# benbergner/ips

Measured on AMD Instinct MI355X. Metric: patches scored/sec (no-grad IPS loop), higher is better.
Workload: dtype f32; 1 GPU; Megapixel-MNIST 1500: 2500 patches of 1x32x32 per image (BASELINE configs[1]), B=16, M=64, I=64, n_token=4, use_pos, eager; parallelism=single GPU, dedup_blank=False, patch_storage=f32, loop_workgroups_per_image=1

## Files before the change

### ips_amd/csrc/scan_common.h

```cpp
#pragma once

#include <algorithm>
#include <cstdlib>

#include "ipsx_common.h"
#include "ipsx_math.h"
#include "ipsx_rowstats.h"
#include "ipsx_stdorder.h"

namespace ipsx {

typedef float f32x16 __attribute__((ext_vector_type(16)));

struct CandView {
    const float* cl;
    const float* lg;
    const int* cand;
    int R;
    __device__ __forceinline__ float get(int l, int r) const {
        if (cl) return cl[l * (R + 1) + r];
        const size_t row = cand ? (size_t)cand[l] : (size_t)l;
        return lg[row * R + r];
    }
};
// ... 714 lines not shown
    if (wave < nruns) {
        const int idx = wave * 64 + lane;
        mine = wave_sort_desc(idx < L ? src[idx] : 0ull, lane);
        runs[idx] = mine;
    }
    asm volatile("s_waitcnt lgkmcnt(0)\n\ts_barrier" ::: "memory");
    if (wave < nruns && mine != 0ull) {
        int rank = 0;
        int r0 = 0;
        for (; r0 + 8 <= nruns; r0 += 8) rank += rank_in_runs<8>(runs + r0 * 64, mine);
        const int left = nruns - r0;
        if (left >= 4) { rank += rank_in_runs<4>(runs + r0 * 64, mine); r0 += 4; }
        if (nruns - r0 == 3) rank += rank_in_runs<3>(runs + r0 * 64, mine);
        else if (nruns - r0 == 2) rank += rank_in_runs<2>(runs + r0 * 64, mine);
        else if (nruns - r0 == 1) rank += rank_in_runs<1>(runs + r0 * 64, mine);
        dst[rank] = mine;
    }
}

__device__ __forceinline__ void lds_barrier() { asm volatile("s_waitcnt lgkmcnt(0)\n\ts_barrier" ::: "memory"); }

#define FAST_STAMP(k)                                                              \
    do {                                                                           \
        if (STAMP) {                                                               \
            const unsigned long long t_ = __builtin_amdgcn_s_memtime();            \
            if (tid == 0) { tacc[k] += t_ - tlast; }                               \
            tlast = t_;                                                            \
        }                                                                          \
    } while (0)

__device__ __attribute__((noinline)) void tie_order_slow(uint64_t* sorted, uint64_t* other, int L, int m, int* stk) {
    torch_tie_order<SCAN_NT>(sorted, other, L, m, stk, threadIdx.x);
}

template <int R>
__device__ __forceinline__ void fold_row_max(uint32_t key, uint32_t* dst, int lane) {
    if (R <= 8) key = max(key, lane_xor_u32<8>(key, lane));
    if (R <= 16) key = max(key, lane_xor_u32<16>(key, lane));
    key = max(key, lane_xor_u32<32>(key, lane));
    if (lane < R && key != 0u) atomicMax(dst + lane, key);
}

__device__ __attribute__((noinline)) void exp_column(const float* xcol, float* ecol, int L, int ld, float mx) {
    for (int l = threadIdx.x; l < L; l += blockDim.x) ecol[l * ld] = det_expf_np(xcol[l * ld] - mx);
}

__device__ __attribute__((noinline)) void exp_column_part(const float* xcol, float* ecol, int L, int ld, float mx, int t0, int nt) {
    for (int l = t0; l < L; l += nt) ecol[l * ld] = det_expf_np(xcol[l * ld] - mx);
}

template <bool PERSIST>
__device__ __forceinline__ float scan_load(const float* p) {
    if (PERSIST) return __hip_atomic_load(p, __ATOMIC_RELAXED, __HIP_MEMORY_SCOPE_AGENT);
    return *p;
}

#define SCAN_WAIT_ROWS(need)                                                                                   \
    do {                                                                                                       \
        if (PERSIST && (long long)(need) > ready_known) {                                                      \
            if (wave == 0) {                                                                                   \
                unsigned long long t0_ = __builtin_amdgcn_s_memrealtime();                                     \
                int v_ = __hip_atomic_load(a.ready + b * a.ready_stride, __ATOMIC_RELAXED, __HIP_MEMORY_SCOPE_AGENT); \
                int seen_ = -1;                                                                                \
                while (v_ >= 0 && v_ < (need)) {                                                               \
                    __builtin_amdgcn_s_sleep(16);                                                              \
                    int w_ = lane < a.ready_words ? __hip_atomic_load(a.ready + lane, __ATOMIC_RELAXED, __HIP_MEMORY_SCOPE_AGENT) : 0; \
                    for (int o_ = 32; o_ >= 1; o_ >>= 1) w_ += __shfl_xor(w_, o_, 64);                         \
                    const unsigned long long now_ = __builtin_amdgcn_s_memrealtime();                          \
                    if (w_ != seen_) { seen_ = w_; t0_ = now_; }                                               \
                    if (now_ - t0_ > a.wait_ticks) { v_ = -1; break; }                                         \
                    v_ = __hip_atomic_load(a.ready + b * a.ready_stride, __ATOMIC_RELAXED, __HIP_MEMORY_SCOPE_AGENT); \
                }                                                                                              \
                if (lane == 0) ccount[6] = v_;                                                     \
            }                                                                                                  \
            lds_barrier();                                                                                     \
             \
             \
            __builtin_amdgcn_fence(__ATOMIC_ACQUIRE, "agent");                                                 \
            ready_known = ccount[6];                                                               \
            if (ready_known < 0) {                                                                             \
                if (tid == 0) { __hip_atomic_fetch_or(a.status, 1, __ATOMIC_RELAXED, __HIP_MEMORY_SCOPE_AGENT); a.plog[5] += 1; } \
                return;                                                                                        \
            }                                                                                                  \
        }                                                                                                      \
    } while (0)

template <int N, int J>
__device__ __forceinline__ uint32_t cmpx32(uint32_t s, uint32_t dir, int lane) {
    const uint32_t o = lane_xor_u32<J>(s, lane);
    const uint32_t c = (uint32_t)__builtin_amdgcn_sbfe((int)dir, N, 1);
    uint32_t d;
    asm("v_med3_u32 %0, %1, %2, %3" : "=v"(d) : "v"(s), "v"(o), "v"(c));
    return d;
}

__device__ __forceinline__ uint32_t sort_directions(int lane) {
    constexpr int KJ[21][2] = {{2, 1}, {4, 2}, {4, 1}, {8, 4}, {8, 2}, {8, 1}, {16, 8}, {16, 4}, {16, 2}, {16, 1}, {32, 16}, {32, 8},
                               {32, 4}, {32, 2}, {32, 1}, {64, 32}, {64, 16}, {64, 8}, {64, 4}, {64, 2}, {64, 1}};
    uint32_t d = 0u;
#pragma unroll
    for (int n = 0; n < 21; ++n) d |= ((((lane & KJ[n][0]) == 0) == ((lane & KJ[n][1]) == 0)) ? 1u : 0u) << n;
    return d;
}

__device__ __forceinline__ uint32_t wave_sort_desc_u32(uint32_t s, uint32_t dir, int lane) {
    s = cmpx32<0, 1>(s, dir, lane);
    s = cmpx32<1, 2>(s, dir, lane); s = cmpx32<2, 1>(s, dir, lane);
    s = cmpx32<3, 4>(s, dir, lane); s = cmpx32<4, 2>(s, dir, lane); s = cmpx32<5, 1>(s, dir, lane);
    s = cmpx32<6, 8>(s, dir, lane); s = cmpx32<7, 4>(s, dir, lane); s = cmpx32<8, 2>(s, dir, lane); s = cmpx32<9, 1>(s, dir, lane);
    s = cmpx32<10, 16>(s, dir, lane); s = cmpx32<11, 8>(s, dir, lane); s = cmpx32<12, 4>(s, dir, lane); s = cmpx32<13, 2>(s, dir, lane);
    s = cmpx32<14, 1>(s, dir, lane);
    s = cmpx32<15, 32>(s, dir, lane); s = cmpx32<16, 16>(s, dir, lane); s = cmpx32<17, 8>(s, dir, lane); s = cmpx32<18, 4>(s, dir, lane);
    s = cmpx32<19, 2>(s, dir, lane); s = cmpx32<20, 1>(s, dir, lane);
    return s;
}

struct TopmArgs {
    int tie_order, stk_off;
    const float* scores;
    int L, m, n2;
    long long* top;
    int* tie;
};

struct ScanCall {
    const float* logits;
    int b;
    int64_t n;
    int m, i, h, n_token;
    int64_t it_begin, it_end;
    int64_t* mem_idx;
    float* mem_score;
    int32_t* tie_flag;
    const int32_t* ready;
    int32_t* status;
    void* workspace;
    size_t workspace_bytes;
    void* stream;
    const int32_t* cond;
    int32_t cond_mask;
    int ready_stride, workgroups;
    int64_t logits_bstride_rows;
};

struct FastPlan {
    bool ok;
    int ept, lch;
    size_t lds;
};
FastPlan scan_fast_plan(int m, int i, int h, int n_token);
int launch_scan_fast(const ScanCall& c, const FastPlan& fp);
bool scan_cam_shape(int m, int i, int h, int n_token);
int launch_scan_cam(const ScanCall& c);
size_t scan_large_ws_per_image(int m, int i, int h, int n_token);
int launch_scan_large(const ScanCall& c);
int scan_large_team(int b, int m, int i, int h, int n_token);
int launch_topm_large(const TopmArgs& a, int b, void* workspace, size_t workspace_bytes, void* stream);
size_t topm_large_ws_per_row(int l);
int scan_large_max_l();

extern int g_persist_wait_ms;
extern bool g_scan_generic;
extern bool g_replay_stamps_on;
extern bool g_scan_direct;
extern bool g_scan_team_trunc;
extern int g_scan_team;
extern bool g_scan_r8;
extern unsigned long long* g_scan_stamps;
unsigned long long* persist_log();

inline int next_pow2(int v) { int p = 1; while (p < v) p <<= 1; return p; }
constexpr size_t kLdsLimit = 160 * 1024;

}
```

### ips_amd/csrc/scorer.hip

```cpp

#include <algorithm>
#include <cstdlib>

#include "scan_common.h"

namespace ipsx {

int g_tie_order = 1;
int g_persist_wait_ms = 50;
bool g_scan_generic = false;
bool g_replay_stamps_on = false;
bool g_scan_team_trunc = true;
int g_scan_team = -1;
bool g_scan_direct = true;
bool g_scan_r8 = true;
unsigned long long* g_scan_stamps = nullptr;

__device__ unsigned long long g_persist_log[8];


unsigned long long* persist_log() {
    static unsigned long long* p[64] = {nullptr};
    int dev = 0;
    if (hipGetDevice(&dev) != hipSuccess || dev < 0 || dev >= 64) dev = 0;
    if (!p[dev]) {
        void* q = nullptr;
        if (hipGetSymbolAddress(&q, HIP_SYMBOL(g_persist_log)) == hipSuccess) p[dev] = static_cast<unsigned long long*>(q);
    }
    return p[dev];
}

}

using namespace ipsx;

IPSX_API int ipsx_scan(const float* logits, int b, int64_t n, int m, int i, int h, int n_token,
                       int64_t* mem_idx, float* mem_score, int32_t* tie_flag, void* workspace, size_t workspace_bytes,
                       void* stream) {
    IPSX_REQUIRE(n > m && i > 0, "scan: needs more patches (%lld) than memory slots (%d)", (long long)n, m);
    if (tie_flag && hipMemsetAsync(tie_flag, 0, sizeof(int32_t) * (size_t)std::max(b, 0), as_stream(stream)) != hipSuccess)
        return fail(IPSX_EHIP, "scan: memset failed");
    return ipsx_scan_range(logits, b, n, m, i, h, n_token, 0, (n - m + i - 1) / i, mem_idx, mem_score, tie_flag,
                           workspace, workspace_bytes, stream);
}

static int scan_range_impl(const float* logits, int b, int64_t n, int m, int i, int h, int n_token,
                           int64_t it_begin, int64_t it_end, int64_t* mem_idx, float* mem_score,
                           int32_t* tie_flag, const int32_t* ready, int32_t* status, void* workspace,
                           size_t workspace_bytes, void* stream, const int32_t* cond = nullptr, int32_t cond_mask = 0,
                           int ready_stride = 0, int workgroups = 0, int64_t logits_bstride_rows = -1);

IPSX_API int ipsx_scan_range(const float* logits, int b, int64_t n, int m, int i, int h, int n_token,
                             int64_t it_begin, int64_t it_end, int64_t* mem_idx, float* mem_score,
                             int32_t* tie_flag, void* workspace, size_t workspace_bytes, void* stream) {
    return scan_range_impl(logits, b, n, m, i, h, n_token, it_begin, it_end, mem_idx, mem_score, tie_flag, nullptr, nullptr,
                           workspace, workspace_bytes, stream);
}

IPSX_API int ipsx_scan_range_strided(const float* logits, int64_t logits_bstride_rows, int b, int64_t n, int m, int i, int h,
                                     int n_token, int64_t it_begin, int64_t it_end, int64_t* mem_idx, float* mem_score,
                                     int32_t* tie_flag, void* workspace, size_t workspace_bytes, void* stream) {
    IPSX_REQUIRE(logits_bstride_rows >= n && logits_bstride_rows < ((int64_t)1 << 31),
                 "scan_range_strided: %lld rows between the images hold %lld candidates (fewer than 2^31)",
                 (long long)logits_bstride_rows, (long long)n);
    return scan_range_impl(logits, b, n, m, i, h, n_token, it_begin, it_end, mem_idx, mem_score, tie_flag, nullptr, nullptr,
                           workspace, workspace_bytes, stream, nullptr, 0, 0, 0, logits_bstride_rows);
}

IPSX_API size_t ipsx_scan_workspace_bytes(int b, int m, int i, int h, int n_token) {
    if (b <= 0 || m <= 0 || i <= 0 || h <= 0 || n_token <= 0) return 0;
    if (scan_fast_plan(m, i, h, n_token).ok && !g_scan_generic) return 0;
    return (size_t)b * scan_large_ws_per_image(m, i, h, n_token);
}

IPSX_API int ipsx_scan_workgroups_per_image(int b, int m, int i, int h, int n_token) {
    if (b <= 0 || m <= 0 || i <= 0 || h <= 0 || n_token <= 0) return 0;
    if (scan_fast_plan(m, i, h, n_token).ok && !g_scan_generic) return 1;
    return scan_large_team(b, m, i, h, n_token);
}

__global__ void publish_rows_kernel(int* ready, int value) {
    __hip_atomic_store(ready, value, __ATOMIC_RELEASE, __HIP_MEMORY_SCOPE_AGENT);
}

IPSX_API int ipsx_scan_persistent_supported(int m, int i, int h, int n_token) {
    if (m <= 0 || i <= 0 || h <= 0 || n_token <= 0) return 0;
    return scan_fast_plan(m, i, h, n_token).ok ? 1 : 0;
}

IPSX_API int ipsx_scan_persistent(const float* logits, int b, int64_t n, int m, int i, int h, int n_token,
                                  int64_t* mem_idx, float* mem_score, int32_t* tie_flag, const int32_t* ready,
                                  int32_t ready_per_image, int32_t* status, void* stream) {
    IPSX_REQUIRE(ready && status, "scan_persistent: needs the progress word(s) and the status word");
    IPSX_REQUIRE(n > m && i > 0, "scan: needs more patches (%lld) than memory slots (%d)", (long long)n, m);
    IPSX_REQUIRE(ipsx_scan_persistent_supported(m, i, h, n_token), "scan_persistent: shape not covered (use ipsx_scan_range)");
    return scan_range_impl(logits, b, n, m, i, h, n_token, 0, (n - m + i - 1) / i, mem_idx, mem_score, tie_flag, ready, status,
                           nullptr, 0, stream, nullptr, 0, ready_per_image ? 1 : 0);
}

IPSX_API int ipsx_scan_persistent_groupable(int m, int i, int h, int n_token) {
    return g_scan_r8 && scan_cam_shape(m, i, h, n_token) ? 1 : 0;
}

IPSX_API int ipsx_scan_persistent_on(const float* logits, int b, int64_t n, int m, int i, int h, int n_token,
                                     int64_t* mem_idx, float* mem_score, int32_t* tie_flag, const int32_t* ready,
                                     int32_t ready_per_image, int32_t* status, int workgroups, void* stream) {
    IPSX_REQUIRE(ready && status, "scan_persistent: needs the progress word(s) and the status word");
    IPSX_REQUIRE(n > m && i > 0, "scan: needs more patches (%lld) than memory slots (%d)", (long long)n, m);
    IPSX_REQUIRE(ipsx_scan_persistent_supported(m, i, h, n_token), "scan_persistent: shape not covered (use ipsx_scan_range)");
    return scan_range_impl(logits, b, n, m, i, h, n_token, 0, (n - m + i - 1) / i, mem_idx, mem_score, tie_flag, ready, status,
                           nullptr, 0, stream, nullptr, 0, ready_per_image ? 1 : 0, workgroups);
}

IPSX_API int ipsx_scan_persistent_ws(const float* logits, int b, int64_t n, int m, int i, int h, int n_token,
                                     int64_t* mem_idx, float* mem_score, int32_t* tie_flag, const int32_t* ready,
                                     int32_t ready_per_image, int32_t* status, int workgroups, void* workspace,
                                     size_t workspace_bytes, void* stream) {
    IPSX_REQUIRE(ready && status, "scan_persistent: needs the progress word(s) and the status word");
    IPSX_REQUIRE(n > m && i > 0, "scan: needs more patches (%lld) than memory slots (%d)", (long long)n, m);
    return scan_range_impl(logits, b, n, m, i, h, n_token, 0, (n - m + i - 1) / i, mem_idx, mem_score, tie_flag, ready, status,
                           workspace, workspace_bytes, stream, nullptr, 0, ready_per_image ? 1 : 0, workgroups);
}

IPSX_API int ipsx_scan_range_if_ws(const float* logits, int b, int64_t n, int m, int i, int h, int n_token,
                                   int64_t it_begin, int64_t it_end, int64_t* mem_idx, float* mem_score,
                                   int32_t* tie_flag, const int32_t* cond, int32_t cond_mask, void* workspace,
                                   size_t workspace_bytes, void* stream) {
    IPSX_REQUIRE(cond && cond_mask, "scan_range_if: needs the condition word and a mask");
    return scan_range_impl(logits, b, n, m, i, h, n_token, it_begin, it_end, mem_idx, mem_score, tie_flag, nullptr, nullptr,
                           workspace, workspace_bytes, stream, cond, cond_mask);
}

__global__ void scan_gate_kernel(const int* status, unsigned long long wait_ticks) {
    const unsigned long long t0 = __builtin_amdgcn_s_memrealtime();
    bool gave_up = false;
    while ((__hip_atomic_load(status, __ATOMIC_RELAXED, __HIP_MEMORY_SCOPE_AGENT) & 2) == 0) {
        __builtin_amdgcn_s_sleep(8);
        if (__builtin_amdgcn_s_memrealtime() - t0 > wait_ticks) { gave_up = true; break; }
    }
    const unsigned long long waited = __builtin_amdgcn_s_memrealtime() - t0;
    g_persist_log[0] += 1;
    g_persist_log[3] = t0;
    if (gave_up) g_persist_log[2] += 1;
    if (waited > g_persist_log[1]) {
        g_persist_log[1] = waited;
        g_persist_log[6] = t0;
        g_persist_log[7] = gave_up ? 0ull : __hip_atomic_load(&g_persist_log[4], __ATOMIC_RELAXED, __HIP_MEMORY_SCOPE_AGENT);
    }
}

IPSX_API int ipsx_scan_gate(const int32_t* status, void* stream) {
    IPSX_REQUIRE(status, "scan_gate: null pointer");
    scan_gate_kernel<<<dim3(1), dim3(1), 0, as_stream(stream)>>>(status, (unsigned long long)g_persist_wait_ms * 100000ull);
    return launched("scan_gate");
}

__global__ void part_wait_kernel(const int* done, int want, int* status, int bit, unsigned long long wait_ticks) {
    unsigned long long t0 = __builtin_amdgcn_s_memrealtime();
    int last = __hip_atomic_load(done, __ATOMIC_RELAXED, __HIP_MEMORY_SCOPE_AGENT);
    while (last < want) {
        __builtin_amdgcn_s_sleep(32);
        const int v = __hip_atomic_load(done, __ATOMIC_RELAXED, __HIP_MEMORY_SCOPE_AGENT);
        const unsigned long long t = __builtin_amdgcn_s_memrealtime();
        if (v != last) { last = v; t0 = t; }
        else if (t - t0 > wait_ticks) {
            __hip_atomic_fetch_or(status, bit, __ATOMIC_RELAXED, __HIP_MEMORY_SCOPE_AGENT);
            break;
        }
    }
    __builtin_amdgcn_fence(__ATOMIC_ACQUIRE, "agent");
}

IPSX_API int ipsx_part_wait(const int32_t* done, int32_t want, int32_t* status, int32_t bit, void* stream) {
    IPSX_REQUIRE(done && status && bit, "part_wait: needs the counter, the status word and a bit");
    part_wait_kernel<<<dim3(1), dim3(1), 0, as_stream(stream)>>>(done, want, status, bit,
                                                                 (unsigned long long)g_persist_wait_ms * 100000ull);
    return launched("part_wait");
}

IPSX_API int ipsx_publish_rows(int32_t* ready, int32_t value, void* stream) {
    IPSX_REQUIRE(ready, "publish_rows: null pointer");
    publish_rows_kernel<<<dim3(1), dim3(1), 0, as_stream(stream)>>>(ready, value);
    return launched("publish_rows");
}

IPSX_API int ipsx_scan_range_if(const float* logits, int b, int64_t n, int m, int i, int h, int n_token,
                                int64_t it_begin, int64_t it_end, int64_t* mem_idx, float* mem_score,
                                int32_t* tie_flag, const int32_t* cond, int32_t cond_mask, void* stream) {
    IPSX_REQUIRE(cond && cond_mask, "scan_range_if: needs the condition word and a mask");
    IPSX_REQUIRE(scan_fast_plan(m, i, h, n_token).ok, "scan_range_if: shapes of the LDS-resident loop only");
    return scan_range_impl(logits, b, n, m, i, h, n_token, it_begin, it_end, mem_idx, mem_score, tie_flag, nullptr, nullptr,
                           nullptr, 0, stream, cond, cond_mask);
}

static int scan_range_impl(const float* logits, int b, int64_t n, int m, int i, int h, int n_token,
                           int64_t it_begin, int64_t it_end, int64_t* mem_idx, float* mem_score,
                           int32_t* tie_flag, const int32_t* ready, int32_t* status, void* workspace,
                           size_t workspace_bytes, void* stream, const int32_t* cond, int32_t cond_mask, int ready_stride,
                           int workgroups, int64_t logits_bstride_rows) {
    IPSX_REQUIRE(logits && mem_idx, "scan: null pointer");
    IPSX_REQUIRE(b > 0 && m > 0 && i > 0 && h > 0 && n_token > 0, "scan: bad sizes");
    IPSX_REQUIRE(n > m, "scan: needs more patches (%lld) than memory slots (%d)", (long long)n, m);
    IPSX_REQUIRE(n < ((int64_t)1 << 31), "scan: too many patches");
    IPSX_REQUIRE(it_begin >= 0 && it_begin <= it_end && it_end <= (n - m + i - 1) / i,
                 "scan: iteration range [%lld, %lld) outside the loop", (long long)it_begin, (long long)it_end);
    if (it_begin == it_end) return IPSX_OK;
    const FastPlan fp = scan_fast_plan(m, i, h, n_token);
    ScanCall c = {logits, b, n, m, i, h, n_token, it_begin, it_end, mem_idx, mem_score, tie_flag, ready, status, workspace,
                  workspace_bytes, stream, cond, cond_mask, ready_stride, workgroups, logits_bstride_rows < 0 ? n : logits_bstride_rows};
    if (!fp.ok || (g_scan_generic && !ready && !cond)) return launch_scan_large(c);
    if (g_scan_r8 && scan_cam_shape(m, i, h, n_token)) return launch_scan_cam(c);
    return launch_scan_fast(c, fp);
}

IPSX_API int ipsx_set_persistent_wait_ms(int ms) {
    const int prev = g_persist_wait_ms;
    if (ms > 0) g_persist_wait_ms = ms > 20000 ? 20000 : ms;
    return prev;
}

IPSX_API int ipsx_set_tie_order(int mode) {
    const int prev = ipsx::g_tie_order;
    if (mode >= 0 && mode <= 2) ipsx::g_tie_order = mode;
    return prev;
}

extern "C" __attribute__((visibility("default"))) int ipsx_dbg_persist_log(unsigned long long* out8) {
    unsigned long long zero[8] = {0, 0, 0, 0, 0, 0, 0, 0};
    if (hipMemcpyFromSymbol(out8, HIP_SYMBOL(ipsx::g_persist_log), sizeof(zero)) != hipSuccess) return -1;
    return hipMemcpyToSymbol(HIP_SYMBOL(ipsx::g_persist_log), zero, sizeof(zero)) == hipSuccess ? 0 : -1;
}

extern "C" __attribute__((visibility("default"))) void ipsx_dbg_scan_stamps(unsigned long long* buf) {
    ipsx::g_scan_stamps = buf;
}

extern "C" __attribute__((visibility("default"))) void ipsx_dbg_scan_generic(int on) { g_scan_generic = on != 0; }

extern "C" __attribute__((visibility("default"))) void ipsx_dbg_scan_direct(int on) { g_scan_direct = on != 0; }
extern "C" __attribute__((visibility("default"))) void ipsx_dbg_scan_team(int w) { g_scan_team = w; }
extern "C" __attribute__((visibility("default"))) void ipsx_dbg_scan_team_trunc(int on) { g_scan_team_trunc = on != 0; }
extern "C" __attribute__((visibility("default"))) void ipsx_dbg_scan_r8(int on) { g_scan_r8 = on != 0; }
```

### ips_amd/dist.py

```python

import math

import torch
import torch.distributed as dist

from . import hip

PARTS = 4
DEFAULT_UNITS = 256

PART_SHARES = (0.5, 0.8, 0.95, 1.0)

PART_SHARES_LOOP_BOUND = (0.15, 0.4, 0.7, 1.0)


def part_iterations(n_iter, parts=PARTS, shares=None):
    P = max(1, min(parts, n_iter))
    shares = shares if shares is not None else PART_SHARES
    shares = shares if P == len(shares) else [(k + 1) / P for k in range(P)]
    its = [0]
    for k in range(P):
        lo = its[-1] + 1
        hi = n_iter - (P - 1 - k)
        its.append(min(max(round(shares[k] * n_iter), lo), hi))
    its[-1] = n_iter
    return its


class LaunchModel:

    REST_STEPS = ((0.25, 0.28), (0.5, 0.54), (0.75, 0.80), (1.0, 1.0))
    BESIDE = 3.5

    def __init__(self, round=0, t_round=0.0, t_row=0.0, t_launch=10.0, t_iter=7.0, t_xchg=60.0, kind="rows"):
        self.round, self.t_round, self.t_row = int(round), float(t_round), float(t_row)
        self.t_launch, self.t_iter, self.t_xchg, self.kind = float(t_launch), float(t_iter), float(t_xchg), kind

    def rounds(self, n):
        if n <= 0 or not self.round:
            return 0.0
        full, rest = divmod(int(n), self.round)
        if rest:
            f = rest / self.round
            full += next(c for lim, c in self.REST_STEPS if f <= lim)
        return float(full)

    def encode_us(self, n):
        if n <= 0:
            return 0.0
        return self.t_launch + (self.rounds(n) * self.t_round if self.round else n * self.t_row)

    def key(self):
        return (self.kind, self.round, round(self.t_round, 3), round(self.t_row, 6), self.t_launch, round(self.t_iter, 3), self.t_xchg)


def default_units():
    if torch.cuda.is_available():
        return hip.device_geometry(torch.device("cuda", torch.cuda.current_device())).cus
    return DEFAULT_UNITS


def loop_iteration_us(M, I, H, T):
    L, R = M + I, H * T
    if L > 1024:
        return 92.0 * L * R / 80000.0
    if (M, I, H, T) == (256, 256, 8, 1):
        return 4.2
    return 2.5 + L * R / 1000.0


_UNIT_FLOPS = 157.3e12 / 256


def _conv_macs(encoder, patch_shape):
    import copy
    macs = [0]

    def hook(m, inp, out):
        macs[0] += out[0].numel() * m.in_channels // m.groups * m.kernel_size[0] * m.kernel_size[1]
    try:
        enc = copy.deepcopy(encoder).to("meta").eval()
        hs = [m.register_forward_hook(hook) for m in enc.modules() if isinstance(m, torch.nn.Conv2d)]
        with torch.no_grad():
            enc(torch.empty((1,) + tuple(patch_shape[-3:]), device="meta"))
        for h in hs:
            h.remove()
    except Exception:
        return 100e6
    return float(macs[0])


def launch_model(net, patch_shape, units=None, precision=None):
    units = int(units or default_units())
    ca = net.transf.crs_attn
    t_iter = loop_iteration_us(net.M, net.I, ca.H, ca.n_token)
    precision = precision or hip.precision()
    if net.is_image and tuple(patch_shape[-3:]) == (1, 32, 32) and len(net.encoder) == 7:
        if precision == "bf16":
            return LaunchModel(round=16 * units, t_round=16 * 256 / 36.0, t_iter=t_iter, kind="fused32:bf16")
        t_round = {"fp32x3": 8 * 256 / 6.8}.get(precision, 8 * 37257216 / (_UNIT_FLOPS * 0.88) * 1e6)
        return LaunchModel(round=8 * units, t_round=t_round, t_iter=t_iter, kind="fused32:" + precision)
    if net.is_image:
        key = ("macs", tuple(patch_shape[-3:]))
        cache = net.__dict__.setdefault("_launch_model_cache", {})
        if key not in cache:
            cache[key] = _conv_macs(net.encoder, patch_shape)
        t_row = 2 * cache[key] / (_UNIT_FLOPS * units * 0.8) * 1e6
        n_conv = sum(1 for m in net.encoder.modules() if isinstance(m, torch.nn.Conv2d))
        return LaunchModel(t_row=t_row, t_launch=8.0 * n_conv, t_iter=t_iter, kind="layers")
    F = int(patch_shape[-1])
    return LaunchModel(t_row=2.0 * F * net.D / (_UNIT_FLOPS * units * 0.75) * 1e6, t_launch=15.0, t_iter=t_iter, kind="rows")


def _plan_cost(its, N, M, I, world, B, model):
    P = len(its) - 1
    done, main = [], 0.0
    for k in range(P):
        e0 = 0 if k == 0 else min(N, M + its[k] * I)
        e1 = N if k == P - 1 else min(N, M + its[k + 1] * I)
        main += model.encode_us(B * -(-(e1 - e0) // world))
        done.append(main)
    side = 0.0
    for k in range(P):
        side = max(side, done[k]) + model.t_xchg
        n = its[k + 1] - its[k]
        slow = model.t_iter * model.BESIDE
        beside = min(n, int(max(0.0, main - side) // slow))
        side += beside * slow + (n - beside) * model.t_iter
    return side


_PLAN_CACHE = {}


def plan_iterations(N, M, I, world, B=1, model=None, parts=PARTS):
    n_iter = math.ceil((N - M) / I)
    if model is None:
        return part_iterations(n_iter, parts)
    key = (N, M, I, world, B, parts, model.key())
    hit = _PLAN_CACHE.get(key)
    if hit is not None:
        return list(hit)
    cands = {tuple(part_iterations(n_iter, p, sh)) for p in range(1, parts + 1)
             for sh in (PART_SHARES, PART_SHARES_LOOP_BOUND, None)}
    if model.round:
        def piece(it0, it1):
            e0 = 0 if it0 == 0 else M + it0 * I
            return B * -(-(min(N, M + it1 * I) - e0) // world)

        def last_fitting(it0, limit):
            e0 = 0 if it0 == 0 else M + it0 * I
            rows = (limit // B) * world
            it1 = min((e0 + rows - M) // I, n_iter - 1)
            return it1 if it1 > it0 else None

        total_rounds = max(1.0, piece(0, n_iter) / model.round)

        def grow(prefix, left):
            cands.add(tuple(prefix + [n_iter]))
            if left <= 1:
                return
            it0 = prefix[-1]
            rest_rounds = piece(it0, n_iter) / model.round
            if rest_rounds <= 0.25:
                return
            limits = set()
            rs = range(0, int(rest_rounds) + 1)
            if len(rs) > 10:
                rs = sorted({int(round(rest_rounds * f)) for f in (0.08, 0.15, 0.25, 0.35, 0.5, 0.65, 0.8, 0.9, 0.95)} |
                            {1, 2, int(rest_rounds) - 1, int(rest_rounds)})
            for r in rs:
                for frac, _ in ((0.0, 0.0),) + (LaunchModel.REST_STEPS[:3] if total_rounds < 6 else ()):
                    lim = int((r + frac) * model.round)
                    if lim > 0:
                        limits.add(lim)
            nxt = {last_fitting(it0, lim) for lim in limits}
            for it1 in sorted(x for x in nxt if x is not None):
                grow(prefix + [it1], left - 1)

        grow([0], parts)
    best = min(cands, key=lambda c: (round(_plan_cost(c, N, M, I, world, B, model), 3), len(c), c))
    _PLAN_CACHE[key] = best
    return list(best)


def partition(N, M, I, world, parts=PARTS, B=1, model=None):
    its = plan_iterations(N, M, I, world, B, model, parts)
    P = len(its) - 1
    edges = [0] + [min(N, M + it * I) for it in its[1:]]
    edges[-1] = N
    piece = [max(1, math.ceil((edges[k + 1] - edges[k]) / world)) for k in range(P)]
    return its, edges, piece


class ShardPlan:

    def __init__(self, N, M, I, world, B=1, model=None, parts=PARTS):
        self.N, self.M, self.I, self.world, self.B, self.model = N, M, I, world, B, model
        self.its, self.edges, self.piece = partition(N, M, I, world, parts, B, model)

    def spans(self, rank):
        out = []
        for k, q in enumerate(self.piece):
            lo = min(self.edges[k] + rank * q, self.edges[k + 1])
            out.append((lo, min(lo + q, self.edges[k + 1])))
        return out

    def indices(self, rank):
        spans = self.spans(rank)
        return torch.cat([torch.arange(lo, hi, dtype=torch.int64) for lo, hi in spans]) if spans else torch.empty(0, dtype=torch.int64)

    def launches(self, rank):
        return [self.B * (hi - lo) for lo, hi in self.spans(rank)]

    def rounds(self, rank=0):
        n = self.launches(rank)
        if self.model is None or not self.model.round:
            return 0.0, 0.0
        return sum(self.model.rounds(v) for v in n), sum(n) / self.model.round

# ... 310 lines not shown
```

### ips_amd/hip.py

```python

import collections
import ctypes as C
import os
import subprocess

import torch

_PKG = os.path.dirname(os.path.abspath(__file__))
_SO = os.path.join(_PKG, "lib", "libipsx.so")
_LIB = None

f32p = C.c_void_p
ABI_MAJOR = 3


def backend():
    b = os.environ.get("IPSX_BACKEND", "hip").lower()
    if b not in ("hip", "aten"):
        raise ValueError("IPSX_BACKEND must be 'hip' or 'aten', got {!r}".format(b))
    return b


def precision():
    p = os.environ.get("IPSX_PRECISION", "fp32").lower()
# ... 618 lines not shown
    if len(tables):
        held, held_rows, piece, dst = tables[0]
        if piece is not None:
            raise ValueError("table 0 is the patch table: its piece is the view (pass None)")
        if dst.dtype != images.dtype or tuple(dst.shape[2:]) != view.patch_shape or dst.device != images.device:
            raise ValueError("table 0: rows of {} {}, the view's patches are {} {}".format(
                dst.dtype, tuple(dst.shape[2:]), images.dtype, view.patch_shape))
    arr, B = _stream_tables(tables, n_cand)
    if sel is not None and (sel.dtype != torch.int64 or tuple(sel.shape) != (B, M) or not sel.is_contiguous()):
        raise ValueError("sel must be a contiguous (B, M) int64 tensor")
    unit = C.c_int(0)
    st = _stream() if images.is_cuda else None
    _ck(lib().ipsx_stream_commit_view(arr, len(tables), _p(images), C.byref(view.struct), images.element_size(), _p(sel), B or 0,
                                      M, n_cand, tail_first, C.byref(unit), st), "ipsx_stream_commit_view")
    return unit.value


def scan_range_if(lg, M, I, H, T, it_begin, it_end, mem_idx, tie, cond, mask=1, workspace=None):
    B, N = lg.shape[:2]
    if workspace is not None:
        _ck(lib().ipsx_scan_range_if_ws(_p(lg), B, N, M, I, H, T, it_begin, it_end, _p(mem_idx), None, _p(tie), _p(cond), mask,
                                        _p(workspace), workspace.numel(), _stream()), "ipsx_scan_range_if_ws")
        return mem_idx
    _ck(lib().ipsx_scan_range_if(_p(lg), B, N, M, I, H, T, it_begin, it_end, _p(mem_idx), None, _p(tie), _p(cond), mask,
                                 _stream()), "ipsx_scan_range_if")
    return mem_idx


Geometry = collections.namedtuple("Geometry", "cus xcds cus_per_xcd")
_GEOMETRY = {}


def device_geometry(dev):
    dev = torch.device(dev)
    idx = dev.index if dev.index is not None else torch.cuda.current_device()
    g = _GEOMETRY.get(idx)
    if g is None:
        props = torch.cuda.get_device_properties(idx)
        cus = int(props.multi_processor_count)
        arch = str(getattr(props, "gcnArchName", ""))
        xcds = cus // 32 if (arch.startswith("gfx95") or arch.startswith("gfx94")) and cus % 32 == 0 and cus >= 32 else 1
        g = _GEOMETRY[idx] = Geometry(cus, xcds, cus // xcds)
    return g


_PERSIST_OK = {}
_PERSIST_OFF = None


def persistent_wait_ms(ms=0):
    return lib().ipsx_set_persistent_wait_ms(int(ms))


_PERSIST_STRIKES = 0
_PERSIST_WAIT_SET = False


def persistent_ok(dev):
    global _PERSIST_WAIT_SET
    if _PERSIST_OFF is not None:
        return False
    if not _PERSIST_WAIT_SET:
        _PERSIST_WAIT_SET = True
        ms = int(os.environ.get("IPSX_PERSIST_WAIT_MS", "0") or 0)
        if ms > 0:
            persistent_wait_ms(ms)
    dev = torch.device(dev)
    idx = dev.index if dev.index is not None else torch.cuda.current_device()
    ok = _PERSIST_OK.get(idx)
    if ok is None:
        ok = _PERSIST_OK[idx] = _persistent_selftest(torch.device("cuda", idx))
    return ok


def persistent_disable(reason):
    global _PERSIST_OFF
    if _PERSIST_OFF is None:
        import warnings
        _PERSIST_OFF = reason
        warnings.warn("ips_amd: persistent selection loops are switched off for this process: " + reason +
                      " (IPSX_SCAN_PERSIST=0 avoids the attempt)")


_PERSIST_CALLS = 0
_PERSIST_RECENT = []


def persistent_timed_out(dev):
    global _PERSIST_STRIKES
    import warnings
    _PERSIST_STRIKES += 1
    limit = max(1, int(os.environ.get("IPSX_PERSIST_STRIKES", "3") or 3))
    window = max(1, int(os.environ.get("IPSX_PERSIST_WINDOW", "1000") or 1000))
    _PERSIST_RECENT[:] = [c for c in _PERSIST_RECENT if _PERSIST_CALLS - c < window] + [_PERSIST_CALLS]
    what = "a persistent selection loop timed out waiting for rows (its call was redone with per-part launches: results valid)"
    if len(_PERSIST_RECENT) >= limit:
        persistent_disable("%s - %d such events within %d calls" % (what, len(_PERSIST_RECENT), window))
        return False
    dev = torch.device(dev)
    idx = dev.index if dev.index is not None else torch.cuda.current_device()
    ok = _PERSIST_OK[idx] = _persistent_selftest(torch.device("cuda", idx))
    if not ok:
        persistent_disable(what + "; a loop beside its producer no longer passes the device's self-test")
        return False
    warnings.warn("ips_amd: %s; the device's self-test passes, the persistent pipelines stay on (event %d of %d allowed within "
                  "%d calls; IPSX_PERSIST_WAIT_MS raises the wait, IPSX_PERSIST_STRIKES the allowance)"
                  % (what, len(_PERSIST_RECENT), limit, window))
    return True


def _persistent_selftest(dev):
    M = I = 16
    H, T = 8, 1
    if not scan_persistent_supported(M, I, H, T):
        return False
    N = M + 4 * I
    with torch.cuda.device(dev):
        lg = torch.zeros((1, N, H * T), dtype=torch.float32, device=dev)
        mem = torch.empty((1, M), dtype=torch.int64, device=dev)
        words = torch.zeros((3,), dtype=torch.int32, device=dev)
        side, main = side_stream(dev), torch.cuda.current_stream(dev)
        side.wait_stream(main)
        with torch.cuda.stream(side):
            scan_persistent(lg, M, I, H, T, mem, words[0:1], words[1:2], words[2:3])
        scan_gate(words[2:3])
        publish_rows(words[1:2], N)
        main.wait_stream(side)
        torch.cuda.synchronize(dev)
        status = int(words[2].item())
    return (status & 1) == 0 and (status & 2) == 2


_SIDE_STREAMS = {}


def side_stream(dev):
    dev = torch.device(dev)
    key = (dev.type, dev.index if dev.index is not None else torch.cuda.current_device())
    st = _SIDE_STREAMS.get(key)
    if st is None:
        st = _SIDE_STREAMS[key] = torch.cuda.Stream(device=dev, priority=-1)
    return st


def scan_persistent_supported(M, I, H, T):
    return bool(lib().ipsx_scan_persistent_supported(M, I, H, T))


def scan_persistent_large(M, I, H, T):
    return (not scan_persistent_supported(M, I, H, T) and lib().ipsx_scan_workspace_bytes(1, M, I, H, T) > 0
            and M + I <= 16384 and H * T <= 256)


def scan_persistent_groupable(M, I, H, T):
    return bool(lib().ipsx_scan_persistent_groupable(M, I, H, T))


def scan_persistent(lg, M, I, H, T, mem_idx, tie, ready, status, workgroups=0, workspace=None, stream=None):
    B, N = lg.shape[:2]
    if not lg.is_contiguous():
        raise ValueError("scan_persistent needs the full contiguous (B, N, H*T) logits buffer")
    if ready.numel() not in (1, B):
        raise ValueError("ready: one word, or one per image")
    st = C.c_void_p(stream.cuda_stream) if stream is not None else _stream()
    if workspace is not None:
        _ck(lib().ipsx_scan_persistent_ws(_p(lg), B, N, M, I, H, T, _p(mem_idx), None, _p(tie), _p(ready),
                                          1 if (ready.numel() == B and B > 1) else 0, _p(status), int(workgroups),
                                          _p(workspace), workspace.numel(), st), "ipsx_scan_persistent_ws")
        return mem_idx
    _ck(lib().ipsx_scan_persistent_on(_p(lg), B, N, M, I, H, T, _p(mem_idx), None, _p(tie), _p(ready),
                                      1 if (ready.numel() == B and B > 1) else 0, _p(status), int(workgroups), st),
        "ipsx_scan_persistent_on")
    return mem_idx


def scan_gate(status):
    _ck(lib().ipsx_scan_gate(_p(status), _stream()), "ipsx_scan_gate")


def publish_rows(ready, n_rows):
    _ck(lib().ipsx_publish_rows(_p(ready), int(n_rows), _stream()), "ipsx_publish_rows")


def _scores_impl(x, qs, wk, H, Dk, T, want_attn):
    x = _f32(x)
    B, L, D = x.shape
    sc = torch.empty((B, L), dtype=torch.float32, device=x.device)
    attn = torch.empty((B, H, T, L), dtype=torch.float32, device=x.device) if want_attn else None
    nb = lib().ipsx_scores_workspace_bytes(B, L, D, H, T)
    ws = torch.empty(max(nb, 1), dtype=torch.uint8, device=x.device)
    wkp = pack_linear(wk)
    _ck(lib().ipsx_scores(_p(x), _p(wkp), _p(qs), B, L, D, H, Dk, T, _p(sc), _p(attn),
                          _p(ws), nb, _stream()), "ipsx_scores")
    return sc, attn


def scores(x, qs, wk, H, Dk, T):
    return _scores_impl(x, qs, wk, H, Dk, T, False)[0]


def attn_map(x, qs, wk, H, Dk, T):
    return _scores_impl(x, qs, wk, H, Dk, T, True)[1]


def topm(sc, M):
    sc = _f32(sc)
    B, L = sc.shape
    top = torch.empty((B, M), dtype=torch.int64, device=sc.device)
    tie = torch.zeros((B,), dtype=torch.int32, device=sc.device)
    nb = lib().ipsx_topm_workspace_bytes(B, L, M)
    ws = torch.empty(nb, dtype=torch.uint8, device=sc.device) if nb else None
    _ck(lib().ipsx_topm(_p(sc), B, L, M, _p(top), _p(tie), _p(ws), nb, _stream()), "ipsx_topm")
    return top


def gather_rows(src, idx):
    B, M = idx.shape
    if src.stride(0) == 0 and src.shape[0] > 1:
        src = src[:1]
    src = src if src.is_contiguous() else src.contiguous()
    idx = idx if idx.is_contiguous() else idx.contiguous()
    N = src.shape[1]
    row_bytes = src[0, 0].numel() * src.element_size()
    out = torch.empty((B, M) + tuple(src.shape[2:]), dtype=src.dtype, device=src.device)
    bstride = N if src.shape[0] > 1 else 0
    _ck(lib().ipsx_gather_rows(_p(src), _p(idx), _p(out), B, N, M, row_bytes, bstride, _stream()),
        "ipsx_gather_rows")
    return out


def dequant_patches(q, table):
    if q.dtype != torch.uint8 or q.dim() < 3:
        raise TypeError("expected uint8 (..., C, h, w) patches, got {} {}".format(q.dtype, tuple(q.shape)))
    table = _patch_table(table, q.shape[-3], q.device)
    q = q if q.is_contiguous() else q.contiguous()
    out = torch.empty(q.shape, dtype=torch.float32, device=q.device)
    c, hw = q.shape[-3], q.shape[-2] * q.shape[-1]
    _ck(lib().ipsx_dequant_patches(_p(q), _p(table), _p(out), q.numel() // max(1, c * hw), c, hw, _stream()),
        "ipsx_dequant_patches")
    return out


def ips_finish_supported(src, pos):
    if not (on_device(src) and src.is_contiguous() and src.dim() >= 3):
        return False
    if (src[0, 0].numel() * src.element_size()) % 16 or src.data_ptr() % 16:
        return False
    if pos is None:
        return True
    if not on_device(pos) or pos.dim() != 3:
        return False
    p1 = pos[:1] if pos.stride(0) == 0 else pos
    return p1.is_contiguous() and (pos.shape[2] * pos.element_size()) % 16 == 0 and pos.data_ptr() % 16 == 0


def ips_finish(src, pos, idx_buf, status, status_host, order=None):
    B, M = idx_buf.shape
    N = src.shape[1]
    row_bytes = src[0, 0].numel() * src.element_size()
    out = torch.empty((B, M) + tuple(src.shape[2:]), dtype=src.dtype, device=src.device)
    idx = torch.empty_like(idx_buf)
    out_pos = None
    pos_bytes = pos_bs = 0
    if pos is not None:
        pos_bs = 0 if (pos.stride(0) == 0 or pos.shape[0] == 1) else pos.shape[1]
        pos_bytes = pos.shape[2] * pos.element_size()
        out_pos = torch.empty((B, M, pos.shape[2]), dtype=pos.dtype, device=pos.device)
    if order is not None:
        if order.dtype != torch.int64 or order.dim() != 2 or order.shape[1] != N or order.shape[0] not in (1, B) or \
                not order.is_contiguous() or order.device != src.device:
            raise ValueError("order must be a contiguous (B or 1, N) int64 tensor on the patches' device")
        _ck(lib().ipsx_ips_finish_indexed(_p(src), row_bytes, N if src.shape[0] > 1 else 0, N, _p(pos), pos_bytes, pos_bs, _p(idx_buf),
                                          _p(order), N if order.shape[0] > 1 else 0, B, M, _p(out), _p(out_pos), _p(idx), _p(status),
                                          _p(status_host), _stream()), "ipsx_ips_finish_indexed")
        return idx, out, out_pos
    _ck(lib().ipsx_ips_finish(_p(src), row_bytes, N if src.shape[0] > 1 else 0, N, _p(pos), pos_bytes, pos_bs, _p(idx_buf), B, M,
                              _p(out), _p(out_pos), _p(idx), _p(status), _p(status_host), _stream()), "ipsx_ips_finish")
    return idx, out, out_pos


def order_index(order, B, N, out=None):
    if order.dtype != torch.int64 or order.dim() != 2 or order.shape[1] != N or order.shape[0] not in (1, B) or \
            not order.is_contiguous() or not order.is_cuda:
        raise ValueError("order must be a contiguous (B or 1, N) int64 tensor on the device")
    if out is None:
        out = torch.empty((B, N), dtype=torch.int32, device=order.device)
    elif out.dtype != torch.int32 or out.numel() != B * N or not out.is_contiguous() or out.device != order.device:
        raise ValueError("out must be B * N contiguous int32 on the order's device")
    _ck(lib().ipsx_order_index(_p(order), N if order.shape[0] > 1 else 0, B, N, _p(out), _stream()), "ipsx_order_index")
    return out.view(B, N)


def patchify(img, patch_size, patch_stride):
    img = _f32(img)
    B, Cc, H, W = img.shape
    (ph, pw), (sh, sw) = patch_size, patch_stride
    n = lib().ipsx_patchify_count(H, W, ph, pw, sh, sw)
    if n <= 0:
        raise ValueError("patch {}x{} / stride {}x{} does not fit a {}x{} image".format(ph, pw, sh, sw, H, W))
    out = torch.empty((B, n, Cc, ph, pw), dtype=torch.float32, device=img.device)
    _ck(lib().ipsx_patchify(_p(img), B, Cc, H, W, ph, pw, sh, sw, _p(out), _stream()), "ipsx_patchify")
    return out


class PatchView:

# ... 178 lines not shown
```

Baseline: 34.01 million patches/s.

## Add shape-specialized scan kernel for M=I=64, 8 heads x 4 tokens

Adds a dedicated single-workgroup-per-image iterative top-M scan kernel, hard-coded for M=I=64, H=8, T=4 (the Megapixel-MNIST config). Inside the loop it double-buffers the logits and their exponentials in LDS and recomputes exp only for columns whose row max changed. Ranking is a counting sort with 8 threads per key. Half the workgroup prefetches the next chunk while the other half scores. The dispatcher routes matching shapes to it by default, and the loop-time cost model gets a fixed per-iteration estimate for this shape. It adds a large specialized code path that must match the generic kernel's tie-handling semantics.

Result: faster. 38.52 million patches/s, median of 6 (+13.3%).

```diff
diff --git a/ips_amd/csrc/scan_common.h b/ips_amd/csrc/scan_common.h
--- a/ips_amd/csrc/scan_common.h
+++ b/ips_amd/csrc/scan_common.h
@@ -890,6 +890,8 @@
 int launch_scan_fast(const ScanCall& c, const FastPlan& fp);
 bool scan_cam_shape(int m, int i, int h, int n_token);
 int launch_scan_cam(const ScanCall& c);
+bool scan_mnist_shape(int m, int i, int h, int n_token);
+int launch_scan_mnist(const ScanCall& c);
 size_t scan_large_ws_per_image(int m, int i, int h, int n_token);
 int launch_scan_large(const ScanCall& c);
 int scan_large_team(int b, int m, int i, int h, int n_token);
@@ -904,6 +906,7 @@
 extern bool g_scan_team_trunc;
 extern int g_scan_team;
 extern bool g_scan_r8;
+extern bool g_scan_mnist;
 extern unsigned long long* g_scan_stamps;
 unsigned long long* persist_log();
 
diff --git a/ips_amd/csrc/scan_mnist.hip b/ips_amd/csrc/scan_mnist.hip
--- /dev/null
+++ b/ips_amd/csrc/scan_mnist.hip
@@ -0,0 +1,311 @@
+
+#include <algorithm>
+#include <cstdlib>
+
+#include "scan_common.h"
+
+namespace ipsx {
+
+namespace mn {
+constexpr int M = 64, I = 64, L = 128, R = 32, H = 8, T = 4, LD = 36, NT = 1024;
+constexpr int OFF_KEYA = 0;
+constexpr int OFF_SORTED = OFF_KEYA + L * 8;
+constexpr int OFF_CAND = OFF_SORTED + L * 8;
+constexpr int OFF_PMAX = OFF_CAND + 2 * L * 4;
+constexpr int OFF_CNT = OFF_PMAX + 4 * R * 4;
+constexpr int OFF_PREV = OFF_CNT + 32;
+constexpr int OFF_DEN = OFF_PREV + 2 * R * 4;
+constexpr int OFF_X = (OFF_DEN + R * 4 + 15) & ~15;
+constexpr int OFF_E = OFF_X + 2 * L * LD * 4;
+constexpr int OFF_STK = OFF_E + 2 * L * LD * 4;
+constexpr int LDS_BYTES = OFF_STK + STK_BYTES;
+static_assert(OFF_KEYA % 16 == 0 && OFF_X % 16 == 0 && (LD * 4) % 16 == 0, "16-byte rows");
+static_assert(H * T == R && M + I == L && L * 8 == NT, "scan_mnist_kernel: 8 threads per key");
+static_assert(OFF_STK == 77728, "scan_mnist_kernel: 77,728 B of LDS + the replay's scratch (STK_BYTES)");
+static_assert(LDS_BYTES <= 160 * 1024, "scan_mnist_kernel: LDS");
+}
+
+template <int K>
+__device__ __forceinline__ float quad_bcast(float v) {
+    return as_float((uint32_t)__builtin_amdgcn_update_dpp(0, (int)as_u32(v), K * 0x55, 0xF, 0xF, false));
+}
+
+template <bool PERSIST>
+__global__ __launch_bounds__(mn::NT) void scan_mnist_kernel(ScanArgs a) {
+    using namespace mn;
+    extern __shared__ __attribute__((aligned(16))) unsigned char smem[];
+    if (!PERSIST && scan_skipped(a.cond, a.cond_mask)) return;
+    __builtin_amdgcn_s_setprio(3);
+    if (PERSIST) {
+        asm volatile("v_mov_b32 v127, 0" ::: "v127");
+        if (threadIdx.x == 0) {
+            __hip_atomic_fetch_or(a.status, 2, __ATOMIC_RELAXED, __HIP_MEMORY_SCOPE_AGENT);
+            __hip_atomic_store(&a.plog[4], (unsigned long long)__builtin_amdgcn_s_memrealtime(), __ATOMIC_RELAXED, __HIP_MEMORY_SCOPE_AGENT);
+        }
+    }
+    uint64_t* const keyA = reinterpret_cast<uint64_t*>(smem + OFF_KEYA);
+    uint64_t* const sorted = reinterpret_cast<uint64_t*>(smem + OFF_SORTED);
+    uint32_t* const pmax = reinterpret_cast<uint32_t*>(smem + OFF_PMAX);
+    int* const ccount = reinterpret_cast<int*>(smem + OFF_CNT);
+    uint32_t* const prevk = reinterpret_cast<uint32_t*>(smem + OFF_PREV);
+    float* const rden = reinterpret_cast<float*>(smem + OFF_DEN);
+    const int tid = threadIdx.x, lane = tid & 63, wave = tid >> 6;
+    const int b = blockIdx.x;
+    const int r = tid & (R - 1);
+    const int hid = tid - 512;
+    const float* const lg = a.lg + (size_t)b * a.n * R;
+    int ready_known = 0;
+    if (tid < 4 * R) pmax[tid] = 0u;
+    if (tid < 2) ccount[2 + tid] = 0;
+    lds_barrier();
+    SCAN_WAIT_ROWS(std::min<long long>(a.n, a.it0 * (long long)I + M + I));
+    {
+        float* const x0 = reinterpret_cast<float*>(smem + OFF_X);
+        int* const cand0 = reinterpret_cast<int*>(smem + OFF_CAND);
+        uint32_t km = 0u;
+#pragma unroll
+        for (int k = 0; k < 2; ++k) {
+            const int l = (tid >> 5) + 32 * k;
+            const size_t row = a.it0 == 0 ? (size_t)l : (size_t)a.mem_idx[(size_t)b * M + l];
+            const float v = scan_load<PERSIST>(lg + row * R + r);
+            x0[l * LD + r] = v;
+            km = max(km, max_key(v));
+        }
+        fold_row_max<R>(km, pmax, lane);
+        if (tid < M) cand0[tid] = a.it0 == 0 ? tid : (int)a.mem_idx[(size_t)b * M + tid];
+    }
+    const long long n_iter = a.it1 - a.it0;
+    float pf[4];
+    {
+        float* const x0 = reinterpret_cast<float*>(smem + OFF_X);
+        int* const cand0 = reinterpret_cast<int*>(smem + OFF_CAND);
+        const long long lo = a.it0 * (long long)I + M;
+        const int cnt = n_iter > 0 ? (int)std::min<long long>(I, a.n - lo) : 0;
+        uint32_t kc = 0u;
+#pragma unroll
+        for (int k = 0; k < 2; ++k) {
+            const int e = tid + NT * k;
+            if (e < cnt * R) {
+                const float v = scan_load<PERSIST>(lg + (size_t)lo * R + e);
+                x0[(M + (e >> 5)) * LD + r] = v;
+                kc = max(kc, max_key(v));
+            }
+        }
+        fold_row_max<R>(kc, pmax + R, lane);
+        if (tid < cnt) cand0[M + tid] = (int)(lo + tid);
+        const long long lo1 = lo + I;
+        const int cnt1 = n_iter > 1 ? (int)std::max<long long>(0, std::min<long long>(I, a.n - lo1)) : 0;
+        if (cnt1 > 0) SCAN_WAIT_ROWS(lo1 + cnt1);
+#pragma unroll
+        for (int k = 0; k < 4; ++k) {
+            const int e = hid + 512 * k;
+            pf[k] = (hid >= 0 && e < cnt1 * R) ? scan_load<PERSIST>(lg + (size_t)lo1 * R + e) : 0.0f;
+        }
+    }
+    int tie = 0;
+    const int n_it = (int)n_iter, n_rows = (int)a.n;
+    for (int k_it = 0; k_it < n_it; ++k_it) {
+        const int lo = ((int)a.it0 + k_it) * I + M;
+        const int cnt = min(I, n_rows - lo);
+        const int Lc = M + cnt;
+        const int par = k_it & 1;
+        float* const xc = reinterpret_cast<float*>(smem + OFF_X) + par * (L * LD);
+        float* const xn = reinterpret_cast<float*>(smem + OFF_X) + (par ^ 1) * (L * LD);
+        float* const ec = reinterpret_cast<float*>(smem + OFF_E) + par * (L * LD);
+        float* const en = reinterpret_cast<float*>(smem + OFF_E) + (par ^ 1) * (L * LD);
+        int* const cand = reinterpret_cast<int*>(smem + OFF_CAND) + par * L;
+        int* const cnew = reinterpret_cast<int*>(smem + OFF_CAND) + (par ^ 1) * L;
+        uint32_t* const mkey = pmax + 2 * R * par;
+        uint32_t* const mkey_nx = pmax + 2 * R * (par ^ 1);
+        const int lo1 = lo + I;
+        const int cnt1 = k_it + 1 < n_it ? max(0, min(I, n_rows - lo1)) : 0;
+        lds_barrier();
+        if (tid == 0) ccount[2 + (par ^ 1)] = 0;
+        const uint32_t mbits = as_u32(max_key_value(max(mkey[r], mkey[R + r])));
+        const float rowmax = as_float(mbits);
+        const bool changed = k_it == 0 || prevk[par * R + r] != mbits;
+        if (tid < R) prevk[(par ^ 1) * R + r] = mbits;
+        {
+            unsigned long long moved = __ballot(changed) & 0xFFFFFFFFull;
+            if (moved != 0ull) {
+                if (__popcll(moved) >= 8) {
+                    if (changed) {
+#pragma unroll
+                        for (int k = 0; k < 4; ++k) {
+                            const int l = (tid >> 5) + 32 * k;
+                            if (l < Lc) ec[l * LD + r] = det_expf_np(xc[l * LD + r] - rowmax);
+                        }
+                    }
+                } else {
+                    while (moved) {
+                        const int rr = __ffsll((long long)moved) - 1;
+                        moved &= moved - 1ull;
+                        exp_column(xc + rr, ec + rr, Lc, LD, __shfl(rowmax, rr, 64));
+                    }
+                }
+                lds_barrier();
+            }
+        }
+        {
+            const float* const col = ec + lane * LD + wave;
+            const float a0 = col[0], a1 = col[64 * LD], b0 = col[16], b1 = col[64 * LD + 16];
+            const bool has1 = lane + 64 < Lc;
+            float s0 = 0.0f, s1 = 0.0f;
+            s0 = s0 + a0; s1 = s1 + b0;
+            s0 = s0 + (has1 ? a1 : 0.0f); s1 = s1 + (has1 ? b1 : 0.0f);
+            wave_sum2(s0, s1, lane);
+            if (lane == 0) { rden[wave] = 1.0f / s0; rden[wave + 16] = 1.0f / s1; }
+        }
+        lds_barrier();
+        if (tid < 2 * R) mkey[tid] = 0u;
+        if (wave < 8) {
+            const int l = tid >> 2, t = tid & 3;
+            const float* const er = ec + l * LD + t;
+            float ev[H], dn[H];
+#pragma unroll
+            for (int hh = 0; hh < H; ++hh) { ev[hh] = er[hh * T]; dn[hh] = rden[hh * T + t]; }
+            float sh = 0.0f;
+#pragma unroll
+            for (int hh = 0; hh < H; ++hh) sh = sh + ev[hh] * dn[hh];
+            const float q = l < Lc ? sh / (float)H : 0.0f;
+            float st = 0.0f;
+            st = st + quad_bcast<0>(q); st = st + quad_bcast<1>(q); st = st + quad_bcast<2>(q); st = st + quad_bcast<3>(q);
+            if (t == 0) keyA[l] = l < Lc ? rank_key(st / (float)T, (uint32_t)l) : 0ull;
+        } else {
+            uint32_t kc = 0u;
+#pragma unroll
+            for (int k = 0; k < 4; ++k) {
+                const int row = (hid >> 5) + 16 * k;
+                if (row < cnt1) {
+                    xn[(M + row) * LD + r] = pf[k];
+                    en[(M + row) * LD + r] = det_expf_np(pf[k] - rowmax);
+                    kc = max(kc, max_key(pf[k]));
+                }
+            }
+            fold_row_max<R>(kc, mkey_nx + R, lane);
+            if (hid < cnt1) cnew[M + hid] = (int)(lo1 + hid);
+        }
+        lds_barrier();
+        {
+            const int kk = tid >> 3, p = tid & 7;
+            const uint64_t mine = keyA[kk];
+            const ulonglong2* const kp = reinterpret_cast<const ulonglong2*>(keyA) + p;
+            ulonglong2 v[8];
+#pragma unroll
+            for (int i = 0; i < 8; ++i) v[i] = kp[8 * i];
+            uint32_t c = 0u;
+#pragma unroll
+            for (int i = 0; i < 8; ++i) c += (v[i].x > mine ? 1u : 0u) + (v[i].y > mine ? 1u : 0u);
+            c += lane_xor_u32<1>(c, lane);
+            c += lane_xor_u32<2>(c, lane);
+            c += lane_xor_u32<4>(c, lane);
+            if (p == 0 && mine != 0ull) sorted[c] = mine;
+        }
+        lds_barrier();
+        {
+            const uint32_t* const sw = reinterpret_cast<const uint32_t*>(sorted);
+            const unsigned long long eqm = __ballot(sw[2 * lane + 1] == sw[2 * lane + 3]);
+            if (eqm != 0ull) {
+                if (a.tie_order != 0) {
+                    bool hit = false;
+                    for (int j = tid; j < M && !hit; j += NT)
+                        for (int k = j + 1; k < Lc && !hit && (sorted[k] >> 32) == (sorted[j] >> 32); ++k) {
+                            bool same = true;
+                            if (a.tie_order == 1) {
+                                const uint4* ra = reinterpret_cast<const uint4*>(xc + key_pos(sorted[j]) * LD);
+                                const uint4* rb = reinterpret_cast<const uint4*>(xc + key_pos(sorted[k]) * LD);
+                                uint32_t diff = 0u;
+#pragma unroll
+                                for (int rr = 0; rr < R / 4; ++rr) {
+                                    const uint4 va = ra[rr], vb = rb[rr];
+                                    diff |= (va.x ^ vb.x) | (va.y ^ vb.y) | (va.z ^ vb.z) | (va.w ^ vb.w);
+                                }
+                                same = diff == 0u;
+                            }
+                            hit = hit || same;
+                        }
+                    if (__ballot(hit) != 0ull && lane == 0) ccount[2 + par] = 1;
+                }
+                lds_barrier();
+                if (tid == 0 && (eqm >> (M - 1)) != 0ull) tie = 1;
+                if (a.tie_order != 0 && ccount[2 + par] != 0)
+                    tie_order_slow(sorted, keyA, Lc, M, reinterpret_cast<int*>(smem + OFF_STK));
+            }
+        }
+        {
+            const int lo2 = lo + 2 * I;
+            const int cnt2 = k_it + 2 < n_it ? max(0, min(I, n_rows - lo2)) : 0;
+            if (cnt2 > 0) SCAN_WAIT_ROWS(lo2 + cnt2);
+#pragma unroll
+            for (int k = 0; k < 4; ++k) {
+                const int e = hid + 512 * k;
+                pf[k] = (hid >= 0 && e < cnt2 * R) ? scan_load<PERSIST>(lg + (size_t)lo2 * R + e) : 0.0f;
+            }
+        }
+        {
+            const uint32_t* const spos = reinterpret_cast<const uint32_t*>(sorted);
+            if (wave < 8) {
+                uint32_t p[4];
+#pragma unroll
+                for (int k = 0; k < 4; ++k) p[k] = ~spos[2 * ((tid >> 5) + 16 * k)] & (L - 1);
+                float gx[4];
+#pragma unroll
+                for (int k = 0; k < 4; ++k) gx[k] = xc[p[k] * LD + r];
+                uint32_t km = 0u;
+#pragma unroll
+                for (int k = 0; k < 4; ++k) { xn[((tid >> 5) + 16 * k) * LD + r] = gx[k]; km = max(km, max_key(gx[k])); }
+                fold_row_max<R>(km, mkey_nx, lane);
+            } else {
+                const int j = hid >> 3, qd = (hid & 7) * 4;
+                const uint32_t p = ~spos[2 * j] & (L - 1);
+                const uint32_t pc = ~spos[2 * (hid & (M - 1))] & (L - 1);
+                const float4 ge = *reinterpret_cast<const float4*>(ec + p * LD + qd);
+                const int ci = cand[pc];
+                *reinterpret_cast<float4*>(en + j * LD + qd) = ge;
+                if (hid < M) cnew[hid] = ci;
+            }
+        }
+    }
+    lds_barrier();
+    {
+        const int parn = (int)(n_iter & 1);
+        const int* const cand = reinterpret_cast<const int*>(smem + OFF_CAND) + parn * L;
+        if (tid < M) {
+            a.mem_idx[(size_t)b * M + tid] = cand[tid];
+            if (a.mem_score) a.mem_score[(size_t)b * M + tid] = n_iter > 0 ? key_score(sorted[tid]) : 0.0f;
+        }
+    }
+    if (a.tie && tid == 0 && tie) a.tie[b] = 1;
+}
+
+bool scan_mnist_shape(int m, int i, int h, int n_token) { return h == mn::H && n_token == mn::T && m == mn::M && i == mn::I; }
+
+int launch_scan_mnist(const ScanCall& c) {
+    IPSX_REQUIRE(scan_mnist_shape(c.m, c.i, c.h, c.n_token) && c.logits_bstride_rows == c.n && (c.workgroups <= 0 || c.workgroups >= c.b),
+                 "scan_mnist_kernel: 8 heads x 4 tokens, M = I = 64, contiguous logits, one workgroup per image");
+    ScanArgs a;
+    a.plog = persist_log();
+    a.lg = c.logits; a.n = c.n; a.lg_bs = c.logits_bstride_rows; a.m = c.m; a.i = c.i; a.h = c.h; a.T = c.n_token; a.n2 = next_pow2(c.m + c.i);
+    a.it0 = c.it_begin; a.it1 = c.it_end;
+    a.mem_idx = reinterpret_cast<long long*>(c.mem_idx); a.mem_score = c.mem_score; a.tie = c.tie_flag;
+    a.ready = c.ready; a.status = c.status; a.ready_stride = c.ready_stride;
+    a.ready_words = c.ready ? (c.ready_stride ? std::min(c.b, 64) : 1) : 0;
+    a.wait_ticks = (unsigned long long)g_persist_wait_ms * 100000ull;
+    a.cond = c.cond; a.cond_mask = c.cond_mask;
+    a.slides = c.b;
+    a.tie_order = g_tie_order;
+    a.use_lds = 1;
+    a.stk_off = mn::OFF_STK;
+    if (a.ready) {
+        (void)hipFuncSetAttribute(reinterpret_cast<const void*>(scan_mnist_kernel<true>), hipFuncAttributeMaxDynamicSharedMemorySize,
+                                  (int)mn::LDS_BYTES);
+        scan_mnist_kernel<true><<<dim3((unsigned)c.b), dim3(mn::NT), mn::LDS_BYTES, as_stream(c.stream)>>>(a);
+    } else {
+        (void)hipFuncSetAttribute(reinterpret_cast<const void*>(scan_mnist_kernel<false>), hipFuncAttributeMaxDynamicSharedMemorySize,
+                                  (int)mn::LDS_BYTES);
+        scan_mnist_kernel<false><<<dim3((unsigned)c.b), dim3(mn::NT), mn::LDS_BYTES, as_stream(c.stream)>>>(a);
+    }
+    return launched("scan");
+}
+
+}
diff --git a/ips_amd/csrc/scorer.hip b/ips_amd/csrc/scorer.hip
--- a/ips_amd/csrc/scorer.hip
+++ b/ips_amd/csrc/scorer.hip
@@ -14,6 +14,7 @@
 int g_scan_team = -1;
 bool g_scan_direct = true;
 bool g_scan_r8 = true;
+bool g_scan_mnist = true;
 unsigned long long* g_scan_stamps = nullptr;
 
 __device__ unsigned long long g_persist_log[8];
@@ -210,6 +211,9 @@
                   workspace_bytes, stream, cond, cond_mask, ready_stride, workgroups, logits_bstride_rows < 0 ? n : logits_bstride_rows};
     if (!fp.ok || (g_scan_generic && !ready && !cond)) return launch_scan_large(c);
     if (g_scan_r8 && scan_cam_shape(m, i, h, n_token)) return launch_scan_cam(c);
+    if (g_scan_mnist && scan_mnist_shape(m, i, h, n_token) && c.logits_bstride_rows == n && (workgroups <= 0 || workgroups >= b) &&
+        g_scan_stamps == nullptr)
+        return launch_scan_mnist(c);
     return launch_scan_fast(c, fp);
 }
 
@@ -241,3 +245,7 @@
 extern "C" __attribute__((visibility("default"))) void ipsx_dbg_scan_team(int w) { g_scan_team = w; }
 extern "C" __attribute__((visibility("default"))) void ipsx_dbg_scan_team_trunc(int on) { g_scan_team_trunc = on != 0; }
 extern "C" __attribute__((visibility("default"))) void ipsx_dbg_scan_r8(int on) { g_scan_r8 = on != 0; }
+extern "C" __attribute__((visibility("default"))) void ipsx_dbg_scan_mnist(int on) { g_scan_mnist = on != 0; }
+extern "C" __attribute__((visibility("default"))) int ipsx_dbg_scan_mnist_shape(int m, int i, int h, int n_token) {
+    return scan_mnist_shape(m, i, h, n_token) ? 1 : 0;
+}
diff --git a/ips_amd/dist.py b/ips_amd/dist.py
--- a/ips_amd/dist.py
+++ b/ips_amd/dist.py
@@ -60,12 +60,17 @@
     return DEFAULT_UNITS
 
 
+LOOP_US_MNIST = 3.4
+
+
 def loop_iteration_us(M, I, H, T):
     L, R = M + I, H * T
     if L > 1024:
         return 92.0 * L * R / 80000.0
     if (M, I, H, T) == (256, 256, 8, 1):
         return 4.2
+    if (M, I, H, T) == (64, 64, 8, 4):
+        return LOOP_US_MNIST
     return 2.5 + L * R / 1000.0
 
 
diff --git a/ips_amd/hip.py b/ips_amd/hip.py
--- a/ips_amd/hip.py
+++ b/ips_amd/hip.py
@@ -794,6 +794,18 @@
             and M + I <= 16384 and H * T <= 256)
 
 
+def scan_mnist_shape(M, I, H, T):
+    fn = lib().ipsx_dbg_scan_mnist_shape
+    fn.restype, fn.argtypes = C.c_int, [C.c_int] * 4
+    return bool(fn(M, I, H, T))
+
+
+def dbg_scan_mnist(on):
+    fn = lib().ipsx_dbg_scan_mnist
+    fn.restype, fn.argtypes = None, [C.c_int]
+    fn(1 if on else 0)
+
+
 def scan_persistent_groupable(M, I, H, T):
     return bool(lib().ipsx_scan_persistent_groupable(M, I, H, T))
 
```
